# zahraamselim/compressed-rag-suite

Hardware: AMD Instinct MI355X
Metric: queries/sec over N-vector corpus (exact cosine top-k; Recall@10 vs the exact fp32 ranking) (higher is better)
Workload: dtype f16 x f16 -> f32; 1 GPU; c4; corpus_rows=10000000, rows_per_gpu=10000000, dim=384, queries_per_batch=64, distinct_queries_in_flight=2048, lanes=1 encoder + 1 search (encoder kernels <= 48 KB of LDS); 4 batches per sweep, batches_per_encoder_forward=16, searches_per_graph=4, top_k=10, k_scan=24, slab=f16, refine_fp32=True, exact_escalation=True, encoder_in_step=True, engine=rag._engine.RetrievalEngine (the object ContextRetriever.retrieve_batch drives), encoder=all-MiniLM-L6-v2 shape, seeded random weights

## Files before the change

### compressed-rag-suite_amd/csrc/capi.hip

```cpp
#include "../../include/crs_hip.h"

#include <hip/hip_runtime.h>
#include <stdio.h>
#include <string.h>

#include "plan.h"
#include "scan.h"

namespace crs {
int device_cus() {
  static int cus[64] = {0};
  int dev = 0;
  if (hipGetDevice(&dev) != hipSuccess) return 0;
  if (dev < 0 || dev >= 64) return 256;
  if (cus[dev] == 0) {
    hipDeviceProp_t p;
    if (hipGetDeviceProperties(&p, dev) != hipSuccess) return 0;
    cus[dev] = p.multiProcessorCount > 0 ? p.multiProcessorCount : 256;
  }
  return cus[dev];
}
}

namespace {
// ... 54 lines not shown
  const hipError_t e = hipGetLastError();
  return e == hipSuccess ? CRS_OK : hip_fail(e, what);
}
}

extern "C" {

const char* crs_last_error(void) { return g_err; }
int crs_abi_version(void) { return 3; }
int crs_row_elems(int dim, int slab_type) { return crs::row_elems(dim, slab_type); }
int crs_padded_dim(int dim) { return crs_row_elems(dim, CRS_SLAB_F16); }

int crs_scan_workspace_bytes(int nq, int dim, int k, int64_t n_rows, size_t* bytes) {
  if (!bytes) return fail(CRS_EINVAL, "null pointer");
  const char* why = "";
  const int rc = crs::plan_workspace_bytes(nq, dim, k, n_rows, device_cus(), crs::knobs_from_env(), bytes, &why);
  return rc ? fail(rc, "%s", why) : CRS_OK;
}

static int run_scan(const Plan& p, const void* q16, const void* slab, const float* scales, int64_t n_rows, const ScanWs& ws, hipStream_t st) {
  if (p.share_tau) {
    const hipError_t me = hipMemsetAsync(ws.tau, 0, ws.tau_bytes, st);
    if (me != hipSuccess) return (int)me;
  }
  crs::ScanArgs a;
  a.q = reinterpret_cast<const _Float16*>(q16);
  a.slab = slab;
  a.scales = scales;
  a.part_scores = ws.part_s;
  a.part_rows = ws.part_r;
  a.tau_shared = p.share_tau ? ws.tau : nullptr;
  a.stamps = nullptr;
  a.n_rows = (int)n_rows;
  a.n_tiles = p.n_tiles;
  a.nq = p.nq;
  a.k = p.k;
  a.sched = p.sched;
  a.boot = p.boot;
  a.kp = p.kp;
  a.nwg = p.nwg;
  a.nqb = p.nqb;
  a.ticket = p.ticket ? ws.tau : nullptr;
  a.t_dyn = p.t_dyn;
  a.dyn_mask = p.dyn_mask;
  a.nt = p.nt;
  a.no_stagger = p.no_stagger;
  a.no_defer = p.no_defer;
  if (p.ticket) {
    const int ze = crs::scan_ticket_zero(a.ticket, st);
    if (ze) return ze;
  }
  switch (p.family) {
    case crs::Family::W1: return crs::scan_launch_w1(a, p.pdim, st);
    case crs::Family::Wide: return crs::scan_launch_wide(a, p.pdim, p.waves, p.mfma, st);
    default: break;
  }
  if (p.slab_type == CRS_SLAB_I8) return crs::scan_launch_i8(a, p.pdim, p.slots, st);
  return p.family == crs::Family::TileBest ? crs::scan_launch_tb(a, p.pdim, p.waves, p.slots, st) : crs::scan_launch_f16(a, p.pdim, p.variant, st);
}

static int search_args_ok(const Plan& p, const void* q16_dev, const void* slab_dev, const float* scales_dev,
                          const void* workspace_dev, size_t workspace_bytes, const void* out_scores_dev, const void* out_ids_dev) {
  if (!q16_dev || !slab_dev || !workspace_dev || !out_scores_dev || !out_ids_dev)
    return fail(CRS_EINVAL, "null pointer");
  if (p.slab_type == CRS_SLAB_I8 && !scales_dev) return fail(CRS_EINVAL, "int8 slab needs scales");
  if (((uintptr_t)q16_dev | (uintptr_t)slab_dev) & 15) return fail(CRS_EINVAL, "q/slab must be 16-byte aligned");
  if (workspace_bytes < ws_bytes(p)) return fail(CRS_ENOSPC, "workspace too small");
  return CRS_OK;
}

int crs_cosine_topk(const void* q16_dev, int nq, int dim, int slab_type, const void* slab_dev,
                    const float* scales_dev, int64_t n_rows, int k, int64_t id_base,
                    void* workspace_dev, size_t workspace_bytes, float* out_scores_dev,
                    int64_t* out_ids_dev, void* stream) {
  if (slab_type != CRS_SLAB_F16 && slab_type != CRS_SLAB_I8) return fail(CRS_EINVAL, "bad slab_type");
  Plan p;
  int rc = plan_for(nq, dim, k, n_rows, slab_type, &p);
  if (rc) return rc;
  rc = search_args_ok(p, q16_dev, slab_dev, scales_dev, workspace_dev, workspace_bytes, out_scores_dev, out_ids_dev);
  if (rc) return rc;
  hipStream_t st = (hipStream_t)stream;
  ScanWs w = scan_ws(workspace_dev, p);
  int e = run_scan(p, q16_dev, slab_dev, scales_dev, n_rows, w, st);
  if (e == -1) return fail(CRS_EINVAL, "unsupported padded dimension");
  if (e) return hip_fail((hipError_t)e, "scan launch");
  if ((size_t)crs::merge_slices(p.nwg, p.kp) > crs::inter_lists(p.part_elems, nq)) w.inter_s = nullptr;
  if (!p.group_best()) {
    e = crs::merge_launch_i32(w.part_s, w.part_r, p.nwg, nq, p.kp, k, id_base, out_scores_dev, out_ids_dev, w.inter_s, w.inter_i, st);
    if (e) return hip_fail((hipError_t)e, "merge launch");
    return CRS_OK;
  }
  e = crs::merge_launch_i32(w.part_s, w.part_r, p.nwg, nq, p.kp, k, 0, w.win_s, w.win_i, w.inter_s, w.inter_i, st);
  if (e) return hip_fail((hipError_t)e, "merge launch");
  e = (slab_type == CRS_SLAB_I8)
          ? crs::refine_i8_launch(reinterpret_cast<const _Float16*>(q16_dev), nq, p.pdim, slab_dev, scales_dev, (int)n_rows, w.win_s,
                                  w.win_i, k, p.tile_rows, id_base, out_scores_dev, out_ids_dev, st)
          : crs::refine_launch(reinterpret_cast<const _Float16*>(q16_dev), nq, p.pdim, reinterpret_cast<const _Float16*>(slab_dev),
                               (int)n_rows, w.win_s, w.win_i, k, p.tile_rows, id_base, out_scores_dev, out_ids_dev, st);
  if (e == -1) return fail(CRS_EINVAL, "unsupported padded dimension");
  if (e) return hip_fail((hipError_t)e, "refine launch");
  return CRS_OK;
}

int crs_merge_topk(const float* scores_dev, const int64_t* ids_dev, int nlists, int nq, int k_in,
                   int k_out, float* out_scores_dev, int64_t* out_ids_dev, void* stream) {
  if (nlists <= 0 || nq <= 0 || k_in <= 0 || k_out <= 0 || k_out > CRS_MAX_K) return fail(CRS_EINVAL, "bad sizes (k_out <= CRS_MAX_K)");
  if (!scores_dev || !ids_dev || !out_scores_dev || !out_ids_dev) return fail(CRS_EINVAL, "null pointer");
// ... 521 lines not shown
```

### compressed-rag-suite_amd/csrc/plan.cpp

```cpp
#include "plan.h"

#include <stdio.h>
#include <stdlib.h>

#include "../../include/crs_hip.h"

namespace crs {
namespace {

bool env_on(const char* name) {
  const char* e = getenv(name);
  return !(e && e[0] == '0');
}
int env_digit(const char* name, int hi, int dflt) {
  const char* e = getenv(name);
  return (e && e[0] >= '0' && e[0] <= '0' + hi) ? e[0] - '0' : dflt;
}

Knobs read_once() {
  Knobs kn;
  kn.scan_tb = env_on("CRS_SCAN_TB");
  kn.long_chain = env_on("CRS_SCAN_LONG_CHAIN");
  kn.scan_wide = env_on("CRS_SCAN_WIDE");
  kn.scan_w1 = env_on("CRS_SCAN_W1");
  kn.scan_variant = env_digit("CRS_SCAN_VARIANT", 3, 3);
  kn.share_tau = env_digit("CRS_SCAN_SHARE_TAU", 1, 0) == 1;
  kn.scan_boot = env_on("CRS_SCAN_BOOT");
  kn.scan_sched = env_digit("CRS_SCAN_SCHED", 2, 2);
  return kn;
}

size_t align_up(size_t x, size_t a) { return (x + a - 1) / a * a; }

int partial_width(const Knobs& kn, int k) { return (kn.share_tau && k <= 16) ? 16 : k; }

void lay_out(Plan* p, int64_t n_rows, int cus, int tile_rows, int wg_per_cu, int queries) {
  p->tile_rows = tile_rows;
  p->n_tiles = (int)((n_rows + tile_rows - 1) / tile_rows);
  p->nqb = (p->nq + queries - 1) / queries;
  int streams = cus * wg_per_cu / p->nqb;
  if (streams < 1) streams = 1;
  if (p->nqb > 1 && streams >= 8) streams &= ~7;
  p->nwg = p->n_tiles < streams ? p->n_tiles : streams;
  if (p->nqb > 1 && p->nwg >= 8) p->nwg &= ~7;
}
int tiles_per_stream(const Plan& p) { return (p.n_tiles + p.nwg - 1) / p.nwg; }

int tile_best_slots(const Plan& p, const Knobs& kn) {
  const int tps = tiles_per_stream(p);
  if ((size_t)tps * p.nwg <= 8192 && tps <= 2 * scan_wide_slots(p.k)) return 0;
  if (p.k <= 16) return scan_wide_slots(p.k);
  const int slots = !kn.long_chain ? 0
                    : p.slab_type == CRS_SLAB_I8 ? scan_i8_long_chain_slots(p.pdim, p.k) : scan_tb_long_chain_slots(p.pdim, p.waves, p.k);
  return slots > 0 ? slots : -1;
}

int finish_plan(Plan* p, int64_t n_rows, const Knobs& kn) {
  const bool tile_best = p->family == Family::TileBest, wide = p->family == Family::Wide;
  p->part_elems = (size_t)p->nwg * p->nq * p->kp;
  p->share_tau = kn.share_tau;
  const size_t slab_bytes = (size_t)n_rows * p->pdim * (p->slab_type == CRS_SLAB_I8 ? 1 : 2);
  const bool streamed = tile_best || (wide && scan_wide_streamed(p->k));
  p->nt = !streamed ? 0 : kn.scan_nt >= 0 ? kn.scan_nt : (slab_bytes >= ((size_t)1 << 30) && p->nqb == 1);
  const bool tb_chain = tile_best && p->slots > 0 && !(p->slab_type == CRS_SLAB_I8 && p->pdim > 768);
  const bool wide_chain = wide && scan_wide_streamed(p->k) && kn.wide_dyn;
  const int rounds = p->n_tiles / p->nwg;
  p->ticket = (tb_chain || wide_chain) && p->nqb == 1 && !kn.share_tau && kn.tb_dyn > 0 &&
              rounds >= (kn.tb_dyn_min < 4 ? 4 : kn.tb_dyn_min);
  p->t_dyn = p->n_tiles;
  p->dyn_mask = 0;
  if (p->ticket) {
    int stat = (int)((int64_t)rounds * (100 - kn.tb_dyn) / 100);
    if (stat < 2) stat = 2;
    p->t_dyn = stat * p->nwg;
    p->dyn_mask = kn.tb_dyn_g - 1;
  }
  p->boot = (kn.scan_boot && rounds < 24) ? 1 : 0;
  p->sched = kn.scan_sched;
  p->no_stagger = (wide && !kn.wide_stagger) ? 1 : 0;
  p->no_defer = (wide && !kn.wide_defer) ? 1 : 0;
  p->mfma = !wide ? 0 : !wide_has_16(p->pdim, p->waves, p->slots) ? 32 : kn.wide_mfma ? kn.wide_mfma : wide_default_mfma(p->pdim, p->slots);
  return CRS_OK;
}

}

Knobs knobs_from_env() {
  static const Knobs once = read_once();
  Knobs kn = once;
  if (const char* e = getenv("CRS_TB_DYN")) { const int v = atoi(e); kn.tb_dyn = v < 0 ? 0 : v > 100 ? 100 : v; }
  if (const char* e = getenv("CRS_TB_DYN_G")) { const int v = atoi(e); kn.tb_dyn_g = v >= 16 ? 16 : v >= 8 ? 8 : v >= 4 ? 4 : v >= 2 ? 2 : 1; }
  if (const char* e = getenv("CRS_TB_DYN_MIN")) kn.tb_dyn_min = atoi(e);
  kn.wide_dyn = env_on("CRS_WIDE_DYN");
  kn.scan_nt = env_digit("CRS_SCAN_NT", 1, -1);
  kn.fused_tail = env_on("CRS_FUSED_TAIL");
  kn.wide_stagger = env_on("CRS_WIDE_STAGGER");
  kn.wide_defer = env_on("CRS_WIDE_DEFER");
  const char* me = getenv("CRS_WIDE_MFMA");
  kn.wide_mfma = !me ? 0 : (me[0] == '1' && me[1] == '6' && !me[2]) ? 16 : (me[0] == '3' && me[1] == '2' && !me[2]) ? 32 : 0;
  return kn;
}

bool Plan::form_exists() const {
  switch (family) {
    case Family::W1: return w1_form_exists(pdim);
    case Family::Wide: return wide_form_exists(pdim, waves, slots, mfma);
    case Family::TileBest: return slab_type == CRS_SLAB_I8 ? i8_form_exists(pdim, slots) : tb_form_exists(pdim, waves, slots);
    default: return slab_type == CRS_SLAB_I8 ? i8_form_exists(pdim, -1) : classic_form_exists(pdim, classic_list_slots(k));
  }
}

int make_plan(int nq, int dim, int k, int64_t n_rows, int slab_type, int cus, const Knobs& kn, Plan* p, const char** why) {
  const auto bad = [&](int code, const char* msg) { *why = msg; return code; };
  if (nq <= 0 || dim <= 0 || dim > 1024) return bad(CRS_EINVAL, "nq must be > 0 and 0 < dim <= 1024");
  if (k <= 0 || k > CRS_MAX_K) return bad(CRS_EINVAL, "k must be in 1..CRS_MAX_K");
  if (n_rows <= 0 || n_rows > 0x7fffffffLL - 64) return bad(CRS_EINVAL, "n_rows must be in 1..2^31-65");
  if (cus <= 0) return bad(CRS_EHIP, "no HIP device available");
  const bool f16 = slab_type == CRS_SLAB_F16;
  const int pdim = row_elems(dim, slab_type);
  *p = Plan{};
  p->slab_type = slab_type;
  p->nq = nq;
  p->k = k;
  p->pdim = pdim;
  p->variant = kn.scan_variant;

  if (kn.scan_tb && kn.scan_w1 && f16 && nq > 64 && w1_form_exists(pdim)) {
    p->family = Family::W1;
    p->waves = 8;
    lay_out(p, n_rows, cus, kW1TileRows, kW1WgPerCu, kW1Queries);
    p->kp = tiles_per_stream(*p);
    if (p->kp <= kW1MaxDump) return finish_plan(p, n_rows, kn);
  }
  if (kn.scan_tb && kn.scan_wide && f16 && nq > 64 && wide_serves(k, pdim)) {
    p->family = Family::Wide;
    p->waves = nq > 128 ? 8 : 4;
    p->slots = scan_wide_slots(k);
    lay_out(p, n_rows, cus, scan_wide_tile_rows(p->waves, pdim), scan_wide_wg_per_cu(p->waves), wide_queries(p->waves));
    p->kp = 2 * p->slots;
    return finish_plan(p, n_rows, kn);
  }
  if (kn.scan_tb) {
    p->family = Family::TileBest;
    if (f16) {
      p->waves = (nq > 64 && k <= 16 && scan_tb_has_8_waves(pdim)) ? 8 : 4;
      lay_out(p, n_rows, cus, tb_tile_rows(pdim), tb_wg_per_cu(pdim, p->waves), tb_queries(p->waves));
    } else {
      p->waves = 4;
      lay_out(p, n_rows, cus, i8_tile_rows(), classic_wg_per_cu(kn.scan_variant), kI8Queries);
    }
// ... 60 lines not shown
```

### compressed-rag-suite_amd/csrc/plan.h

```cpp
#pragma once
#include <stddef.h>
#include <stdint.h>

#include "scan_forms.h"

namespace crs {

struct Knobs {
  bool scan_tb = true;
  bool long_chain = true;
  bool scan_wide = true;
  bool scan_w1 = true;
  int scan_variant = 3;
  bool share_tau = false;
  bool scan_boot = true;
  int scan_sched = 2;
  int tb_dyn = 85;
  int tb_dyn_g = 8;
  int tb_dyn_min = 96;
  bool wide_dyn = true;
  int scan_nt = -1;
  bool fused_tail = true;
  bool wide_stagger = true;
  bool wide_defer = true;
  int wide_mfma = 0;
};
Knobs knobs_from_env();

constexpr int kW1MaxDump = 256;

struct Plan {
  Family family;
  int slab_type;
  int nq, k;
  int pdim, tile_rows, n_tiles;
  int nwg;
  int nqb;
  int kp;
  int waves;
  int slots;
  int variant;
  bool share_tau;
  int nt;
  bool ticket;
  int t_dyn, dyn_mask;
  int boot, sched;
  int no_stagger;
  int no_defer;
  int mfma;
  size_t part_elems;
  bool group_best() const { return family != Family::Classic; }
  bool form_exists() const;
};

int make_plan(int nq, int dim, int k, int64_t n_rows, int slab_type, int cus, const Knobs& kn, Plan* p, const char** why);
int plan_describe(const Plan& p, char* buf, size_t cap);

struct WsLayout {
  size_t tau, part_s, part_r, win_s, win_i, inter_s, inter_i;
  size_t tau_bytes, bytes;
};
size_t inter_lists(size_t part_elems, int nq);
WsLayout ws_layout(size_t part_elems, int nq, int k);
int plan_workspace_bytes(int nq, int dim, int k, int64_t n_rows, int cus, const Knobs& kn, size_t* bytes, const char** why);

}
```

### compressed-rag-suite_amd/csrc/scan.h

```cpp
#pragma once
#include <hip/hip_runtime.h>
#include <stdint.h>

#include "scan_forms.h"

namespace crs {

int set_error(int code, const char* msg);
int launch_status(const char* what);

struct ScanArgs {
  const _Float16* q;
  const void* slab;
  const float* scales;
  float* part_scores;
  int* part_rows;
  unsigned* tau_shared;
  unsigned long long* stamps;
  int n_rows;
  int n_tiles;
  int nq;
  int k;
  int sched;
  int boot;
  int kp;
  int nwg;
  int nqb;
  unsigned* ticket;
  int t_dyn;
  int dyn_mask;
  int nt;
  int no_stagger;
  int no_defer;
};

struct ExactWs {
  float* thr;
  int* cnt;
  int* done;
  int64_t* lists;
};

int refine_launch(const _Float16* q16, int nq, int pdim, const _Float16* slab, int n_rows, const float* win_s,
                  const int64_t* win, int k, int tile_rows, int64_t id_base, float* out_s, int64_t* out_i, hipStream_t stream);

int refine_i8_launch(const _Float16* q16, int nq, int pdim, const void* slab, const float* scales, int n_rows, const float* win_s,
                     const int64_t* win, int k, int tile_rows, int64_t id_base, float* out_s, int64_t* out_i, hipStream_t stream);

int scan_launch_f16(const ScanArgs& a, int pdim, int variant, hipStream_t stream);
int scan_launch_i8(const ScanArgs& a, int pdim, int slots, hipStream_t stream);
int scan_launch_tb(const ScanArgs& a, int pdim, int nw, int slots, hipStream_t stream);
int scan_ticket_zero(unsigned* ticket, hipStream_t stream);
int scan_launch_wide(const ScanArgs& a, int pdim, int nw, int mfma, hipStream_t stream);
int scan_launch_w1(const ScanArgs& a, int pdim, hipStream_t stream);

int merge_slices(int nlists, int k_in);
int merge_launch_i32(const float* scores, const int* rows, int nlists, int nq, int k_in, int k_out,
                     int64_t id_base, float* out_scores, int64_t* out_ids, float* inter_s, int64_t* inter_i, hipStream_t stream);
int merge_launch_i64(const float* scores, const int64_t* ids, int nlists, int nq, int k_in, int k_out,
                     float* out_scores, int64_t* out_ids, hipStream_t stream);

int merge_launch_wire(const void* wire, size_t block_bytes, size_t scores_off, int nlists, int nq, int k_in, int k_out,
                      float* out_scores, int64_t* out_ids, hipStream_t stream);

int merge_sorted_launch_i64(const float* scores, const int64_t* ids, int nlists, int nq, int k_in, int k_out, float* out_scores,
                            int64_t* out_ids, hipStream_t stream);
int merge_sorted_launch_wire(const void* wire, size_t block_bytes, size_t scores_off, int nlists, int nq, int k_in, int k_out,
                             float* out_scores, int64_t* out_ids, hipStream_t stream);

int mmr_order_launch(const float* vecs, int64_t n_rows, int dim, const int64_t* rows, const double* rel, const int* counts, int nq,
                     int m_max, double lam, int* order, hipStream_t stream);

int rerank_lexical_launch(const float* scores, const int64_t* rows, int nq, int m_max, const int64_t* doc_off, const int* doc_tok,
                          int64_t n_rows, int64_t n_doc_tok, const int64_t* q_off, const int* q_tok, int64_t n_q_tok, const int* q_norm,
                          int k, double threshold, int* order, int* out_count, double* sim, double* rr, int* reranked, hipStream_t stream);

size_t bm25_workspace_bytes(int nq, int k, int64_t n_rows);
int bm25_topk_launch(const int64_t* doc_off, const int* doc_tok, const int* doc_tf, const int* doc_len, int64_t n_rows, int64_t n_doc_tok,
                     const int64_t* q_off, const int* q_tok, const float* q_w, int nq, int n_pairs, float c0, float c1, float k1p1, int k,
                     void* workspace, float* out_s, int64_t* out_i, hipStream_t stream);

int fuse_rrf_launch(const int64_t* dense, int m_dense, const int64_t* lex, int m_lex, int nq, double c, double w_dense, double w_lex,
                    int k_out, int64_t* out_rows, double* out_fused, int* out_dpos, int* out_lpos, int* out_count, hipStream_t stream);

int wordpiece_encode_launch(const uint8_t* text, const int64_t* offsets, int n_texts, int64_t n_bytes, const uint32_t* table,
                            int64_t table_len, const uint32_t* rep, int64_t rep_len, const int32_t* slots, int64_t n_slots,
                            const uint32_t* pool, int64_t pool_len, int max_probe, int lmax, int mode, int unk, int cls, int sep, int pad,
                            int hash_lo, int hash_span, int max_len, int* ids, int* lens, int* flags, hipStream_t stream);
int unigram_encode_launch(const uint8_t* text, const int64_t* offsets, int n_texts, int64_t n_bytes, const uint32_t* table,
                          int64_t table_len, const uint32_t* rep, int64_t rep_len, const int32_t* slots, const double* slot_scores,
                          int64_t n_slots, const uint32_t* pool, int64_t pool_len, int max_probe, int lmax, double unk_score, int opts,
                          int unk, int cls, int sep, int pad, int max_len, int* ids, int* lens, int* flags, hipStream_t stream);

int token_match_launch(const float* a, const int* len_a, int seq_a, const float* b, const int* len_b, int seq_b, int n_pairs, int hidden,
                       const float* w_a, const float* w_b, float* out, hipStream_t stream);

int pairs_above_launch(const void* slab, int pdim, int64_t a_first, int64_t a_rows, int64_t b_first, int64_t b_rows, float thr,
                       int64_t* pairs_out, float* scores_out, int64_t cap, int64_t* counter, hipStream_t stream);
int pairs_verify_launch(const int64_t* pairs, int64_t m, const float* shadow, int64_t n_rows, int d, float thr, int64_t* rows_a,
                        int64_t* rows_b, float* sims, int64_t* counter, hipStream_t stream);

int refine_f32_launch(const float* q32, int nq, int dim, const float* shadow, int64_t n_rows, int64_t id_base,
                      const int64_t* cand, int k_in, int k_out, float* out_s, int64_t* out_i, hipStream_t stream);
int score_rows_launch(const float* q32, int nq, int dim, const float* shadow, int64_t n_rows, int64_t id_base, int k, const int64_t* ids,
                      float* scores, hipStream_t stream);
int rescore_launch(const float* q32, int nq, int dim, const float* shadow, int64_t n_rows,
// ... 24 lines not shown
```

### compressed-rag-suite_amd/csrc/scan_forms.h

```cpp
#pragma once

namespace crs {

enum class Family { Classic, TileBest, Wide, W1 };

constexpr int kSlabF16 = 0, kSlabI8 = 1;

constexpr int row_elems(int dim, int slab_type) {
  const int g = slab_type == kSlabI8 ? 256 : 128;
  return dim <= 0 ? 0 : (dim + g - 1) / g * g;
}
constexpr bool f16_row(int pdim) { return pdim >= 128 && pdim <= 1024 && pdim % 128 == 0; }

constexpr int classic_wg_per_cu(int variant) { return variant == 1 ? 1 : 2; }
constexpr int classic_tile_rows(int pdim) { return pdim <= 512 ? 32 : 16; }
constexpr int classic_list_slots(int k) { return k <= 16 ? 16 : 32; }
constexpr int kClassicQueries = 64;
constexpr bool classic_form_exists(int pdim, int list_slots) { return f16_row(pdim) && (list_slots == 16 || list_slots == 32); }

constexpr int tb_tile_rows(int pdim) { return classic_tile_rows(pdim); }
constexpr bool scan_tb_has_8_waves(int pdim) { return pdim != 640 && pdim != 896; }
constexpr int tb_wg_per_cu(int pdim, int nw) { return nw == 8 ? (pdim <= 384 ? 2 : 1) : (pdim <= 128 ? 3 : 2); }
constexpr int tb_queries(int nw) { return 16 * nw; }
constexpr int scan_wide_slots(int k) { return k <= 4 ? 4 : k <= 10 ? 10 : k <= 16 ? 16 : k <= 24 ? 24 : 32; }
constexpr int scan_tb_long_chain_slots(int pdim, int nw, int k) {
  if (nw != 4 || k <= 16 || k > 64) return 0;
  if (k <= 24) return 24;
  if (k <= 32) return 32;
  if (pdim == 256) return 64;
  if (pdim == 384) return k <= 48 ? 48 : (k <= 56 ? 56 : 0);
  if (pdim == 512 || pdim == 640) return k <= 48 ? 48 : 0;
  if (pdim == 768) return k <= 40 ? 40 : 0;
  return 0;
}
constexpr bool tb_form_exists(int pdim, int nw, int slots) {
  if (!f16_row(pdim) || !(nw == 4 || (nw == 8 && scan_tb_has_8_waves(pdim)))) return false;
  if (slots == 0 || slots == 4 || slots == 10 || slots == 16) return true;
  return slots > 16 && scan_tb_long_chain_slots(pdim, nw, slots) == slots;
}

constexpr int i8_tile_rows() { return 32; }
constexpr int kI8Queries = 64;
constexpr int scan_i8_long_chain_slots(int pdim, int k) { return (k <= 16 || k > 48) ? 0 : k <= 32 ? 32 : (pdim <= 768 ? 48 : 0); }
constexpr bool i8_form_exists(int pdim, int slots) {
  if (!(pdim == 256 || pdim == 512 || pdim == 768 || pdim == 1024)) return false;
  if (slots == -1 || slots == 0 || slots == 4 || slots == 10 || slots == 16) return true;
  return slots > 16 && scan_i8_long_chain_slots(pdim, slots) == slots;
}

constexpr bool wide_serves(int k, int pdim) { return k <= 32 && pdim <= 512 && !(k > 16 && pdim > 384); }
constexpr int scan_wide_tile_rows(int nw, int pdim) { return (nw == 8 && pdim <= 384) ? 64 : 32; }
constexpr int scan_wide_wg_per_cu(int nw) { return nw == 8 ? 1 : 2; }
constexpr int wide_queries(int nw) { return 32 * nw; }
constexpr bool scan_wide_streamed(int k) { return scan_wide_slots(k) > 16; }
constexpr bool wide_has_16(int pdim, int nw, int slots) { return nw == 8 && (pdim == 256 || pdim == 384) && slots > 16; }
constexpr int wide_default_mfma(int pdim, int slots) { return (pdim == 384 && (slots == 24 || slots == 32)) ? 16 : 32; }
constexpr bool wide_form_exists(int pdim, int nw, int slots, int mfma) {
  if (!(pdim == 128 || pdim == 256 || pdim == 384 || pdim == 512) || !(nw == 4 || nw == 8)) return false;
  if (!(slots == 4 || slots == 10 || slots == 16 || ((slots == 24 || slots == 32) && pdim <= 384))) return false;
  return mfma == 32 || (mfma == 16 && wide_has_16(pdim, nw, slots));
}

constexpr int kW1TileRows = 32, kW1WgPerCu = 1, kW1Queries = 256;
constexpr bool w1_form_exists(int pdim) { return pdim == 768; }

}
```

### compressed-rag-suite_amd/csrc/scan_stream.h

```cpp
#pragma once
#include "scan_common.h"

namespace crs {
namespace {

typedef __attribute__((address_space(3))) void* lds_ptr_t;

__device__ __forceinline__ unsigned tile_lds_wave(char* tile_buf, int wave) {
  return __builtin_amdgcn_readfirstlane((unsigned)(size_t)(lds_ptr_t)tile_buf + (unsigned)wave * 1024u);
}

template <int kT, int kTileBytes, int kLoads>
__device__ __forceinline__ void stream_tile(const char* slab, int tile, int n_full, size_t last_chunk, unsigned dst0,
                                            const unsigned (&src_off)[kLoads], int nt) {
  if (tile < n_full) {
    const char* base = uniform_ptr(slab + (size_t)tile * kTileBytes);
    if (nt) {
#pragma unroll
      for (int j = 0; j < kLoads; ++j) lds_dma16_nt(dst0 + (unsigned)(j * kT * 16), src_off[j], base);
    } else {
#pragma unroll
      for (int j = 0; j < kLoads; ++j) lds_dma16(dst0 + (unsigned)(j * kT * 16), src_off[j], base);
    }
  } else {
#pragma unroll
    for (int j = 0; j < kLoads; ++j) {
      size_t off = (size_t)tile * kTileBytes + src_off[j];
      off = off > last_chunk ? last_chunk : off;
      const char* p = slab + off;
      const unsigned dst = dst0 + (unsigned)(j * kT * 16);
      lds_dma16(dst, p);
    }
  }
}

template <int K>
__device__ __forceinline__ void chain_insert(float (&ts)[K], int (&tr)[K], float x, int xr) {
#pragma unroll
  for (int j = 0; j < K; ++j) {
    const bool c = x > ts[j];
    const float s_old = ts[j];
    const int r_old = tr[j];
    ts[j] = c ? x : s_old;
    tr[j] = c ? xr : r_old;
    x = c ? s_old : x;
    xr = c ? r_old : xr;
  }
}

__device__ __forceinline__ bool ticket_due(bool in_dyn, int tn, int tstep, int t_dyn, int dyn_mask) {
  return in_dyn ? ((tn - t_dyn) & dyn_mask) == dyn_mask : tn + tstep >= t_dyn;
}
__device__ __forceinline__ void ticket_draw(unsigned& tk, bool drawer, unsigned* ticket) {
  const unsigned mask = __builtin_amdgcn_readfirstlane(drawer ? 1u : 0u);
  unsigned long long keep;
  unsigned zero = 0u, one = 1u;
  asm volatile("s_mov_b64 %1, exec\n\ts_mov_b32 exec_lo, %2\n\ts_mov_b32 exec_hi, 0\n\tglobal_atomic_add %0, %3, %4, %5 sc0\n\ts_mov_b64 exec, %1"
               : "+v"(tk), "=&s"(keep) : "s"(mask), "v"(zero), "v"(one), "s"(ticket) : "memory");
}
__device__ __forceinline__ void ticket_publish(int* sh_next, int it, unsigned tk, int t_dyn, int dyn_mask) {
  sh_next[it & 1] = t_dyn + (int)tk * (dyn_mask + 1);
}
__device__ __forceinline__ int ticket_take(const int* sh_next, int it, int tend) {
  const int tnn = __builtin_amdgcn_readfirstlane(sh_next[it & 1]);
  return (unsigned)tnn < (unsigned)tend ? tnn : tend;
}

__device__ __forceinline__ void dump_pad(float* part_s, int* part_r, size_t o, int first, int kp) {
  for (int p = first; p < kp; p += 4) {
    part_s[o + p] = kNegInf;
    part_r[o + p] = -1;
  }
}
template <int K>
__device__ __forceinline__ void chain_store(float* part_s, int* part_r, size_t o, const float (&ts)[K], const int (&tr)[K]) {
#pragma unroll
  for (int j = 0; j < K; ++j) {
    part_s[o + j] = ts[j];
    part_r[o + j] = tr[j];
  }
}

template <auto kKernel>
int launch_scan(int lds, int threads, const ScanArgs& a, hipStream_t stream) {
  static bool done = false;
  if (!done) {
    hipError_t e = hipFuncSetAttribute(reinterpret_cast<const void*>(kKernel), hipFuncAttributeMaxDynamicSharedMemorySize, lds);
    if (e != hipSuccess) return (int)e;
    done = true;
  }
  hipLaunchKernelGGL(kKernel, dim3(a.nqb * a.nwg), dim3(threads), lds, stream, a);
  return (int)hipGetLastError();
}

}
}
```

### compressed-rag-suite_amd/csrc/scan_wide.hip

```cpp


#include "scan_stream.h"

namespace crs {
namespace {

typedef float f32x16 __attribute__((ext_vector_type(16)));

template <int D, int NW>
constexpr int wide_rb() { return scan_wide_tile_rows(NW, D) / 32; }

template <int K>
constexpr bool wide_streamed() { return K > 16; }
template <int K>
constexpr bool wide_split() { return K > 16; }
template <int K>
constexpr int wide_lane_slots() { return wide_split<K>() ? K / 2 : K; }
template <int D, int NW, int K>
constexpr bool wide_stagger() {
  if (D == 384 && NW == 8 && K == 24) return true;
  return NW == 8 && D <= 384 && !(D == 384 && K >= 16) && !(D == 256 && K >= 32);
}
#ifndef CRS_WIDE_DEFER_ALL
#define CRS_WIDE_DEFER_ALL 0
#endif
template <int D, int NW, int K, bool S16>
constexpr bool wide_defer() {
  if (!wide_split<K>() || (!S16 && D == 384 && NW == 8 && K == 24)) return false;
  if (CRS_WIDE_DEFER_ALL) return true;
  return S16 && D == 384 && NW == 8 && K == 24;
}

template <int D, int NW>
struct WCfg {
  static constexpr int kThreadsW = NW * 64;
  static constexpr int kCpr = D / 8;
  static constexpr int RB = wide_rb<D, NW>();
  static constexpr int TR = 32 * RB;
  static constexpr int kTileBytes = TR * D * 2;
  static constexpr int kLoads = kTileBytes / (kThreadsW * 16);
  static constexpr int kKsteps = D / 16;
  static constexpr int kQStage = NW * 4096;
  static constexpr int kLds = 2 * kTileBytes > kTileBytes + kQStage ? 2 * kTileBytes : kTileBytes + kQStage;
  static_assert(D % 128 == 0, "row length must be a multiple of 128 elements");
  static_assert(kTileBytes % (kThreadsW * 16) == 0, "tile must split into whole 16-byte loads");
};

template <int RB, bool S16>
struct WAcc { f32x16 a[RB]; };
template <int RB>
struct WAcc<RB, true> { f32x4 a[2 * RB][2]; };

template <int D, int NW, int K, bool S16>
__device__ __forceinline__ void scan_wide_body(const ScanArgs a) {
  using C = WCfg<D, NW>;
  static_assert(!S16 || wide_has_16(D, NW, K), "the 16x16x32 form exists for the split-list forms of 64-row tiles only");
  constexpr int kT = C::kThreadsW;
  extern __shared__ __attribute__((aligned(16))) char smem[];
  char* tile_buf = smem;
  const int tid = threadIdx.x;
  const int lane = tid & 63;
  const int wave = __builtin_amdgcn_readfirstlane(tid >> 6);
  const int nwg = CRS_NSTREAMS;
  const int qblock = CRS_QBLOCK, stream = CRS_STREAM;
  WP_DECL;
  const bool wave_active = (qblock * (NW * 32) + wave * 32) < a.nq;

  unsigned src_off[C::kLoads];
#pragma unroll
  for (int j = 0; j < C::kLoads; ++j) {
    const int P = j * kT + tid;
    const int r = P / C::kCpr, cp = P % C::kCpr;
    src_off[j] = (unsigned)(r * C::kCpr + ((cp & ~15) | ((cp ^ r) & 15))) * 16u;
  }
  const char* slab = reinterpret_cast<const char*>(a.slab);
  const size_t last_chunk = (size_t)a.n_rows * (D * 2) - 16;
  constexpr int RB = C::RB, WTR = C::TR;
  const int n_full = a.n_rows / WTR;
  const unsigned lds_wave = tile_lds_wave(tile_buf, wave);
  auto dma_tile = [&](int tile, int buf) {
    stream_tile<kT, C::kTileBytes>(slab, __builtin_amdgcn_readfirstlane(tile), n_full, last_chunk,
                                   lds_wave + (unsigned)(buf * C::kTileBytes), src_off, wide_streamed<K>() ? a.nt : 0);
  };

  __shared__ int sh_next[2];
  constexpr bool kDyn = wide_streamed<K>();
  const int tend = a.n_tiles;
  const int t_dyn = kDyn ? a.t_dyn : a.n_tiles;
  int t = stream, t_prev = stream;
  int tn = t + nwg;
  dma_tile(t, 0);

  constexpr int KS16 = D / 32;
  const int kq = lane >> 4;
  const int qn = S16 ? (lane & 15) : (lane & 31), h = S16 ? (kq & 1) : (lane >> 5);
  const int qi = qblock * (NW * 32) + wave * 32 + (S16 ? 16 * (kq >> 1) : 0) + qn;
  const bool q_valid = qi < a.nq;
  f16x8 qf[C::kKsteps];
  {
    constexpr int kBlocks = C::kCpr / 8;
    constexpr int kGroup = 3;
    char* qs = tile_buf + C::kTileBytes + wave * 4096;
    const int q0 = qblock * (NW * 32) + wave * 32;
    const char* qbytes = reinterpret_cast<const char*>(a.q);
    const f16x8 z = {0, 0, 0, 0, 0, 0, 0, 0};
#pragma unroll
    for (int g0 = 0; g0 < kBlocks; g0 += kGroup) {
      u32x4 tmp[kGroup * 4];
#pragma unroll
      for (int p = 0; p < kGroup; ++p) {
        if (g0 + p < kBlocks) {
#pragma unroll
          for (int j = 0; j < 4; ++j) {
            const int c = j * 64 + lane, q = c >> 3, col = c & 7;
            const int qq = q0 + q < a.nq ? q0 + q : a.nq - 1;
            tmp[p * 4 + j] = *reinterpret_cast<const u32x4*>(qbytes + (size_t)qq * (D * 2) + (g0 + p) * 128 + col * 16);
          }
        }
      }
#pragma unroll
      for (int p = 0; p < kGroup; ++p) {
        if (g0 + p < kBlocks) {
#pragma unroll
          for (int j = 0; j < 4; ++j) {
            const int c = j * 64 + lane, q = c >> 3, col = c & 7;
            *reinterpret_cast<u32x4*>(qs + q * 128 + ((col ^ ((q >> 1) & 7)) * 16)) = tmp[p * 4 + j];
          }
          if constexpr (S16) {
#pragma unroll
            for (int g = 0; g < 2; ++g) {
              const int row = 16 * g + qn;
#pragma unroll
              for (int kk = 0; kk < 2; ++kk) {
                const int col = 4 * kk + kq;
                const f16x8 v = *reinterpret_cast<const f16x8*>(qs + row * 128 + ((col ^ ((row >> 1) & 7)) * 16));
                qf[g * KS16 + (g0 + p) * 2 + kk] = (q0 + row < a.nq) ? v : z;
              }
            }
          } else {
#pragma unroll
            for (int ksl = 0; ksl < 4; ++ksl) {
              const int col = 2 * ksl + h;
              const f16x8 v = *reinterpret_cast<const f16x8*>(qs + qn * 128 + ((col ^ ((qn >> 1) & 7)) * 16));
              qf[(g0 + p) * 4 + ksl] = q_valid ? v : z;
            }
          }
        }
      }
    }
#pragma unroll
    for (int ks = 0; ks < C::kKsteps; ++ks) {
      f16x8 x = qf[ks];
      asm volatile("" : "+v"(x));
      qf[ks] = x;
    }
// ... 130 lines not shown
#pragma unroll
          for (int rt = 0; rt < 2 * RB; rt += 2) xg[g] = __builtin_fmaxf(__builtin_fmaxf(xg[g], m[rt]), m[rt + 1]);
        } else {
#pragma unroll
          for (int rt = 0; rt < 2 * RB; ++rt) {
            const int row0 = te * WTR + 16 * rt + 4 * kq;
#pragma unroll
            for (int i = 0; i < 4; ++i) xg[g] = (row0 + i < a.n_rows) ? __builtin_fmaxf(xg[g], accs.a[rt][g][i]) : xg[g];
          }
        }
      }
      const auto r0 = __builtin_amdgcn_permlane16_swap(__float_as_uint(xg[0]), __float_as_uint(xg[0]), false, false);
      const auto r1 = __builtin_amdgcn_permlane16_swap(__float_as_uint(xg[1]), __float_as_uint(xg[1]), false, false);
      const float y0 = __builtin_fmaxf(__uint_as_float(r0[0]), __uint_as_float(r0[1]));
      const float y1 = __builtin_fmaxf(__uint_as_float(r1[0]), __uint_as_float(r1[1]));
      const auto rr = __builtin_amdgcn_permlane32_swap(__float_as_uint(y0), __float_as_uint(y1), false, false);
      x = __builtin_fmaxf(__uint_as_float(rr[0]), __uint_as_float(rr[1]));
      pair_tile(x, te * WTR);
    } else {
#pragma unroll
      for (int rb = 0; rb < RB; ++rb) {
        const f32x16& acc = accs.a[rb];
        if (te < n_full) {
          const float m0 = __builtin_fmaxf(__builtin_fmaxf(acc[0], acc[1]), acc[2]);
          const float m1 = __builtin_fmaxf(__builtin_fmaxf(acc[3], acc[4]), acc[5]);
          const float m2 = __builtin_fmaxf(__builtin_fmaxf(acc[6], acc[7]), acc[8]);
          const float m3 = __builtin_fmaxf(__builtin_fmaxf(acc[9], acc[10]), acc[11]);
          const float m4 = __builtin_fmaxf(__builtin_fmaxf(acc[12], acc[13]), acc[14]);
          x = __builtin_fmaxf(x, __builtin_fmaxf(__builtin_fmaxf(__builtin_fmaxf(m0, m1), __builtin_fmaxf(m2, m3)), __builtin_fmaxf(m4, acc[15])));
        } else {
          const int row_base = te * WTR + rb * 32 + 4 * h;
#pragma unroll
          for (int r = 0; r < 16; ++r) {
            const int row = row_base + 8 * (r >> 2) + (r & 3);
            x = (row < a.n_rows) ? __builtin_fmaxf(x, acc[r]) : x;
          }
        }
      }
      x = pair_max(x);
      if constexpr (kSplit) {
        pair_tile(x, te * WTR);
      } else {
        if ((ie & 1) == h) { px = x; pr = te * WTR; }
        if (ie & 1) {
          chain_insert(ts, tr, px, pr);
          px = kNegInf;
          pr = -1;
        }
      }
    }
  };

  int cur = 0, it = 0;
  while (t < tend) {
    const bool has_next = tn < tend;
    if (has_next) dma_tile(tn, cur ^ 1);
    const bool in_dyn = kDyn && tn >= t_dyn;
    const bool draw = kDyn && a.ticket != nullptr && has_next && ticket_due(in_dyn, tn, nwg, t_dyn, a.dyn_mask);
    unsigned tk = 0;
    if constexpr (kDyn) ticket_draw(tk, draw && wave == 0, a.ticket);
    if (wave_active) {
      WP_LAP(1);
      const char* buf = tile_buf + cur * C::kTileBytes;
      if (!late) {
        const Acc acc = sweep(buf);
        WP_LAP(3);
        select(acc, t, it);
      } else {
        if (it > 0) select(acc_prev, t_prev, it - 1);
        WP_LAP(2);
        acc_prev = sweep(buf);
        WP_LAP(3);
      }
    }
    WP_LAP(4);
    int tnn = in_dyn ? tn + 1 : tn + nwg;
    if constexpr (kDyn) {
      asm volatile("s_waitcnt vmcnt(0)" : "+v"(tk) : : "memory");
      if (draw && tid == 0) ticket_publish(sh_next, it, tk, t_dyn, a.dyn_mask);
    } else {
      asm volatile("s_waitcnt vmcnt(0)" ::: "memory");
    }
    WP_LAP(6);
    __syncthreads();
    WP_LAP(7);
    if (kDyn && draw) tnn = ticket_take(sh_next, it, tend);
    cur ^= 1;
    ++it;
    t_prev = t;
    t = tn;
    tn = tnn;
  }

  if (wave_active && late && it > 0) select(acc_prev, t_prev, it - 1);
  if constexpr (kSplit) {
    if constexpr (kDefer) {
      if (wave_active) flush();
    }
    if (wave_active && q_valid) {
      const size_t o = ((size_t)qi * nwg + stream) * a.kp + (size_t)h * KL;
#pragma unroll
      for (int j = 0; j < KL; ++j) {
        a.part_scores[o + j] = ts[j];
        a.part_rows[o + j] = tr[j];
        a.part_scores[o + K + j] = kNegInf;
        a.part_rows[o + K + j] = -1;
      }
    }
  } else {
    if (wave_active && (it & 1)) chain_insert(ts, tr, px, pr);
    if (wave_active && q_valid) {
      const size_t o = ((size_t)qi * nwg + stream) * a.kp + (size_t)h * K;
#pragma unroll
      for (int j = 0; j < K; ++j) {
        a.part_scores[o + j] = ts[j];
        a.part_rows[o + j] = tr[j];
      }
    }
  }
  WP_LAP(10);
  WP_STORE(NW);
}

template <int D, int NW, int K>
__global__ __launch_bounds__(NW * 64, 2) void scan_wide_kernel(const ScanArgs a) {
  scan_wide_body<D, NW, K, false>(a);
}
template <int D, int NW, int K>
__global__ __launch_bounds__(NW * 64, 2) void scan_wide16_kernel(const ScanArgs a) {
  scan_wide_body<D, NW, K, true>(a);
}

template <int D, int NW, int K, bool S16>
int launch_wide(const ScanArgs& a, hipStream_t stream) {
  if constexpr (S16) return launch_scan<&scan_wide16_kernel<D, NW, K>>(WCfg<D, NW>::kLds, NW * 64, a, stream);
  else return launch_scan<&scan_wide_kernel<D, NW, K>>(WCfg<D, NW>::kLds, NW * 64, a, stream);
}

template <int D, int NW, int K>
int launch_wide_if(const ScanArgs& a, int mfma, hipStream_t stream) {
  if constexpr (wide_form_exists(D, NW, K, 16)) {
    if (mfma == 16) return launch_wide<D, NW, K, true>(a, stream);
  }
  if constexpr (wide_form_exists(D, NW, K, 32)) return launch_wide<D, NW, K, false>(a, stream);
  else return -1;
}

template <int D, int NW>
int launch_wide_k(const ScanArgs& a, int mfma, hipStream_t stream) {
  switch (scan_wide_slots(a.k)) {
    case 4: return launch_wide_if<D, NW, 4>(a, mfma, stream);
    case 10: return launch_wide_if<D, NW, 10>(a, mfma, stream);
    case 16: return launch_wide_if<D, NW, 16>(a, mfma, stream);
    case 24: return launch_wide_if<D, NW, 24>(a, mfma, stream);
    default: return launch_wide_if<D, NW, 32>(a, mfma, stream);
  }
}

template <int D>
int launch_wide_d(const ScanArgs& a, int nw, int mfma, hipStream_t stream) {
  return nw == 8 ? launch_wide_k<D, 8>(a, mfma, stream) : launch_wide_k<D, 4>(a, mfma, stream);
}

}

int scan_launch_wide(const ScanArgs& a, int pdim, int nw, int mfma, hipStream_t stream) {
  switch (pdim) {
    case 128: return launch_wide_d<128>(a, nw, mfma, stream);
    case 256: return launch_wide_d<256>(a, nw, mfma, stream);
    case 384: return launch_wide_d<384>(a, nw, mfma, stream);
    case 512: return launch_wide_d<512>(a, nw, mfma, stream);
    default: return -1;
  }
}

}
```

Baseline: 124,300 queries/s.

## Add triple-buffered ring pipeline to the wide scan kernel for pdim 384

Adds a three-buffer ring variant of the wide f16 scan kernel that keeps two tile DMAs in flight instead of one. The ticket-based dynamic scheduling is moved to per-slot shared slots so a tile index can be drawn two steps ahead. The goal is to hide more global-memory latency while streaming the slab. In exchange each workgroup uses more LDS, which may lower occupancy, and the static prefix is raised to at least three rounds. It is enabled by default only for pdim 384, 8 waves, 24 slots and the 16x16 MFMA form, and is compiled in a separate translation unit.

```diff
diff --git a/compressed-rag-suite_amd/csrc/capi.hip b/compressed-rag-suite_amd/csrc/capi.hip
--- a/compressed-rag-suite_amd/csrc/capi.hip
+++ b/compressed-rag-suite_amd/csrc/capi.hip
@@ -130,7 +130,8 @@
   }
   switch (p.family) {
     case crs::Family::W1: return crs::scan_launch_w1(a, p.pdim, st);
-    case crs::Family::Wide: return crs::scan_launch_wide(a, p.pdim, p.waves, p.mfma, st);
+    case crs::Family::Wide:
+      return p.ring ? crs::scan_launch_wide_ring(a, p.pdim, p.waves, p.mfma, st) : crs::scan_launch_wide(a, p.pdim, p.waves, p.mfma, st);
     default: break;
   }
   if (p.slab_type == CRS_SLAB_I8) return crs::scan_launch_i8(a, p.pdim, p.slots, st);
diff --git a/compressed-rag-suite_amd/csrc/plan.cpp b/compressed-rag-suite_amd/csrc/plan.cpp
--- a/compressed-rag-suite_amd/csrc/plan.cpp
+++ b/compressed-rag-suite_amd/csrc/plan.cpp
@@ -1,5 +1,6 @@
 #include "plan.h"
 
+#include <assert.h>
 #include <stdio.h>
 #include <stdlib.h>
 
@@ -65,21 +66,25 @@
   const bool tb_chain = tile_best && p->slots > 0 && !(p->slab_type == CRS_SLAB_I8 && p->pdim > 768);
   const bool wide_chain = wide && scan_wide_streamed(p->k) && kn.wide_dyn;
   const int rounds = p->n_tiles / p->nwg;
+  p->mfma = !wide ? 0 : !wide_has_16(p->pdim, p->waves, p->slots) ? 32 : kn.wide_mfma ? kn.wide_mfma : wide_default_mfma(p->pdim, p->slots);
+  p->ring = wide && kn.wide_ring && wide_ring_form(p->pdim, p->waves, p->slots, p->mfma);
+  p->lds = wide ? scan_wide_lds_bytes(p->pdim, p->waves, p->ring) : 0;
   p->ticket = (tb_chain || wide_chain) && p->nqb == 1 && !kn.share_tau && kn.tb_dyn > 0 &&
               rounds >= (kn.tb_dyn_min < 4 ? 4 : kn.tb_dyn_min);
   p->t_dyn = p->n_tiles;
   p->dyn_mask = 0;
   if (p->ticket) {
     int stat = (int)((int64_t)rounds * (100 - kn.tb_dyn) / 100);
-    if (stat < 2) stat = 2;
+    const int stat_min = p->ring ? 3 : 2;
+    if (stat < stat_min) stat = stat_min;
     p->t_dyn = stat * p->nwg;
     p->dyn_mask = kn.tb_dyn_g - 1;
+    assert(p->t_dyn >= stat_min * p->nwg && p->t_dyn <= p->n_tiles);
   }
   p->boot = (kn.scan_boot && rounds < 24) ? 1 : 0;
   p->sched = kn.scan_sched;
   p->no_stagger = (wide && !kn.wide_stagger) ? 1 : 0;
   p->no_defer = (wide && !kn.wide_defer) ? 1 : 0;
-  p->mfma = !wide ? 0 : !wide_has_16(p->pdim, p->waves, p->slots) ? 32 : kn.wide_mfma ? kn.wide_mfma : wide_default_mfma(p->pdim, p->slots);
   return CRS_OK;
 }
 
@@ -96,6 +101,7 @@
   kn.fused_tail = env_on("CRS_FUSED_TAIL");
   kn.wide_stagger = env_on("CRS_WIDE_STAGGER");
   kn.wide_defer = env_on("CRS_WIDE_DEFER");
+  kn.wide_ring = env_on("CRS_WIDE_RING");
   const char* me = getenv("CRS_WIDE_MFMA");
   kn.wide_mfma = !me ? 0 : (me[0] == '1' && me[1] == '6' && !me[2]) ? 16 : (me[0] == '3' && me[1] == '2' && !me[2]) ? 32 : 0;
   return kn;
diff --git a/compressed-rag-suite_amd/csrc/plan.h b/compressed-rag-suite_amd/csrc/plan.h
--- a/compressed-rag-suite_amd/csrc/plan.h
+++ b/compressed-rag-suite_amd/csrc/plan.h
@@ -24,6 +24,7 @@
   bool wide_stagger = true;
   bool wide_defer = true;
   int wide_mfma = 0;
+  bool wide_ring = true;
 };
 Knobs knobs_from_env();
 
@@ -48,6 +49,8 @@
   int no_stagger;
   int no_defer;
   int mfma;
+  bool ring;
+  int lds;
   size_t part_elems;
   bool group_best() const { return family != Family::Classic; }
   bool form_exists() const;
diff --git a/compressed-rag-suite_amd/csrc/scan.h b/compressed-rag-suite_amd/csrc/scan.h
--- a/compressed-rag-suite_amd/csrc/scan.h
+++ b/compressed-rag-suite_amd/csrc/scan.h
@@ -52,6 +52,7 @@
 int scan_launch_tb(const ScanArgs& a, int pdim, int nw, int slots, hipStream_t stream);
 int scan_ticket_zero(unsigned* ticket, hipStream_t stream);
 int scan_launch_wide(const ScanArgs& a, int pdim, int nw, int mfma, hipStream_t stream);
+int scan_launch_wide_ring(const ScanArgs& a, int pdim, int nw, int mfma, hipStream_t stream);
 int scan_launch_w1(const ScanArgs& a, int pdim, hipStream_t stream);
 
 int merge_slices(int nlists, int k_in);
diff --git a/compressed-rag-suite_amd/csrc/scan_forms.h b/compressed-rag-suite_amd/csrc/scan_forms.h
--- a/compressed-rag-suite_amd/csrc/scan_forms.h
+++ b/compressed-rag-suite_amd/csrc/scan_forms.h
@@ -61,6 +61,19 @@
   return mfma == 32 || (mfma == 16 && wide_has_16(pdim, nw, slots));
 }
 
+#ifndef CRS_WIDE_RING_ALL
+#define CRS_WIDE_RING_ALL 0
+#endif
+constexpr bool wide_ring_form(int pdim, int nw, int slots, int mfma) {
+  if (!wide_form_exists(pdim, nw, slots, mfma) || nw != 8 || slots <= 16) return false;
+  if (CRS_WIDE_RING_ALL) return true;
+  return pdim == 384 && slots == 24 && mfma == 16;
+}
+constexpr int scan_wide_lds_bytes(int pdim, int nw, bool ring) {
+  const int tile = scan_wide_tile_rows(nw, pdim) * pdim * 2, qstage = nw * 4096, nbuf = ring ? 3 : 2;
+  return nbuf * tile > (nbuf - 1) * tile + qstage ? nbuf * tile : (nbuf - 1) * tile + qstage;
+}
+
 constexpr int kW1TileRows = 32, kW1WgPerCu = 1, kW1Queries = 256;
 constexpr bool w1_form_exists(int pdim) { return pdim == 768; }
 
diff --git a/compressed-rag-suite_amd/csrc/scan_stream.h b/compressed-rag-suite_amd/csrc/scan_stream.h
--- a/compressed-rag-suite_amd/csrc/scan_stream.h
+++ b/compressed-rag-suite_amd/csrc/scan_stream.h
@@ -66,6 +66,14 @@
   return (unsigned)tnn < (unsigned)tend ? tnn : tend;
 }
 
+__device__ __forceinline__ void ticket_publish_slot(int* sh_next, int slot, unsigned tk, int t_dyn, int dyn_mask) {
+  sh_next[slot] = t_dyn + (int)tk * (dyn_mask + 1);
+}
+__device__ __forceinline__ int ticket_take_slot(const int* sh_next, int slot, int tend) {
+  const int tnn = __builtin_amdgcn_readfirstlane(sh_next[slot]);
+  return (unsigned)tnn < (unsigned)tend ? tnn : tend;
+}
+
 __device__ __forceinline__ void dump_pad(float* part_s, int* part_r, size_t o, int first, int kp) {
   for (int p = first; p < kp; p += 4) {
     part_s[o + p] = kNegInf;
diff --git a/compressed-rag-suite_amd/csrc/scan_wide.hip b/compressed-rag-suite_amd/csrc/scan_wide.hip
--- a/compressed-rag-suite_amd/csrc/scan_wide.hip
+++ b/compressed-rag-suite_amd/csrc/scan_wide.hip
@@ -30,6 +30,9 @@
   if (CRS_WIDE_DEFER_ALL) return true;
   return S16 && D == 384 && NW == 8 && K == 24;
 }
+
+template <int D, int NW, int K, bool S16>
+constexpr bool wide_ring() { return wide_ring_form(D, NW, K, S16 ? 16 : 32); }
 
 template <int D, int NW>
 struct WCfg {
@@ -42,6 +45,8 @@
   static constexpr int kKsteps = D / 16;
   static constexpr int kQStage = NW * 4096;
   static constexpr int kLds = 2 * kTileBytes > kTileBytes + kQStage ? 2 * kTileBytes : kTileBytes + kQStage;
+  static constexpr int kLdsRing = scan_wide_lds_bytes(D, NW, true);
+  static_assert(kLds == scan_wide_lds_bytes(D, NW, false), "the planner's LDS bytes are the launch's");
   static_assert(D % 128 == 0, "row length must be a multiple of 128 elements");
   static_assert(kTileBytes % (kThreadsW * 16) == 0, "tile must split into whole 16-byte loads");
 };
@@ -51,9 +56,10 @@
 template <int RB>
 struct WAcc<RB, true> { f32x4 a[2 * RB][2]; };
 
-template <int D, int NW, int K, bool S16>
+template <int D, int NW, int K, bool S16, bool RING = false>
 __device__ __forceinline__ void scan_wide_body(const ScanArgs a) {
   using C = WCfg<D, NW>;
+  static_assert(!RING || (wide_ring<D, NW, K, S16>() && wide_streamed<K>()), "no ring kernel for this form");
   static_assert(!S16 || wide_has_16(D, NW, K), "the 16x16x32 form exists for the split-list forms of 64-row tiles only");
   constexpr int kT = C::kThreadsW;
   extern __shared__ __attribute__((aligned(16))) char smem[];
@@ -83,13 +89,16 @@
                                    lds_wave + (unsigned)(buf * C::kTileBytes), src_off, wide_streamed<K>() ? a.nt : 0);
   };
 
-  __shared__ int sh_next[2];
+  __shared__ int sh_next[RING ? 3 : 2];
   constexpr bool kDyn = wide_streamed<K>();
   const int tend = a.n_tiles;
   const int t_dyn = kDyn ? a.t_dyn : a.n_tiles;
   int t = stream, t_prev = stream;
   int tn = t + nwg;
   dma_tile(t, 0);
+  if constexpr (RING) {
+    if (tn < tend) dma_tile(tn, 1);
+  }
 
   constexpr int KS16 = D / 32;
   const int kq = lane >> 4;
@@ -100,7 +109,7 @@
   {
     constexpr int kBlocks = C::kCpr / 8;
     constexpr int kGroup = 3;
-    char* qs = tile_buf + C::kTileBytes + wave * 4096;
+    char* qs = tile_buf + (RING ? 2 : 1) * C::kTileBytes + wave * 4096;
     const int q0 = qblock * (NW * 32) + wave * 32;
     const char* qbytes = reinterpret_cast<const char*>(a.q);
     const f16x8 z = {0, 0, 0, 0, 0, 0, 0, 0};
@@ -337,6 +346,55 @@
   };
 
   int cur = 0, it = 0;
+  if constexpr (RING) {
+    int tnn = tn + nwg;
+    while (t < tend) {
+      const bool has_nn = tnn < tend;
+      const int nbuf = cur ? cur - 1 : 2;
+      const bool in_dyn = tnn >= t_dyn;
+      const bool draw = a.ticket != nullptr && has_nn && ticket_due(in_dyn, tnn, nwg, t_dyn, a.dyn_mask);
+      unsigned tk = 0;
+      ticket_draw(tk, draw && wave == 0, a.ticket);
+      auto issue = [&]() {
+        WP_LAP(6);
+        if (has_nn) dma_tile(tnn, nbuf);
+        WP_LAP(1);
+      };
+      const char* buf = tile_buf + cur * C::kTileBytes;
+      if (!wave_active) {
+        asm volatile("s_waitcnt vmcnt(0)" ::: "memory");
+        issue();
+      } else if (!late) {
+        const Acc acc = sweep(buf);
+        WP_LAP(3);
+        select(acc, t, it);
+        WP_LAP(4);
+        asm volatile("s_waitcnt vmcnt(0)" : "+v"(tk) : : "memory");
+        issue();
+        if (draw && tid == 0) ticket_publish_slot(sh_next, cur, tk, t_dyn, a.dyn_mask);
+      } else {
+        if (it > 0) select(acc_prev, t_prev, it - 1);
+        WP_LAP(2);
+        asm volatile("s_waitcnt vmcnt(0)" ::: "memory");
+        issue();
+        acc_prev = sweep(buf);
+        WP_LAP(3);
+      }
+      int t3 = in_dyn ? tnn + 1 : tnn + nwg;
+      asm volatile("s_waitcnt lgkmcnt(0)" ::: "memory");
+      __builtin_amdgcn_s_barrier();
+      asm volatile("" ::: "memory");
+      WP_LAP(7);
+      if (draw) t3 = ticket_take_slot(sh_next, cur, tend);
+      cur = cur == 2 ? 0 : cur + 1;
+      ++it;
+      t_prev = t;
+      t = tn;
+      tn = tnn;
+      tnn = t3;
+    }
+    asm volatile("s_waitcnt vmcnt(0)" ::: "memory");
+  } else {
   while (t < tend) {
     const bool has_next = tn < tend;
     if (has_next) dma_tile(tn, cur ^ 1);
@@ -376,6 +434,7 @@
     t = tn;
     tn = tnn;
   }
+  }
 
   if (wave_active && late && it > 0) select(acc_prev, t_prev, it - 1);
   if constexpr (kSplit) {
@@ -407,6 +466,11 @@
   WP_STORE(NW);
 }
 
+#ifndef CRS_WIDE_TU
+#define CRS_WIDE_TU 0
+#endif
+
+#if CRS_WIDE_TU != 1
 template <int D, int NW, int K>
 __global__ __launch_bounds__(NW * 64, 2) void scan_wide_kernel(const ScanArgs a) {
   scan_wide_body<D, NW, K, false>(a);
@@ -447,8 +511,44 @@
   return nw == 8 ? launch_wide_k<D, 8>(a, mfma, stream) : launch_wide_k<D, 4>(a, mfma, stream);
 }
 
-}
-
+#endif
+
+#if CRS_WIDE_TU != 0
+namespace ring {
+template <int D, int NW, int K>
+__global__ __launch_bounds__(NW * 64, 2) void scan_wide_kernel(const ScanArgs a) {
+  scan_wide_body<D, NW, K, false, true>(a);
+}
+template <int D, int NW, int K>
+__global__ __launch_bounds__(NW * 64, 2) void scan_wide16_kernel(const ScanArgs a) {
+  scan_wide_body<D, NW, K, true, true>(a);
+}
+}
+
+template <int D, int K>
+int launch_ring_if(const ScanArgs& a, int mfma, hipStream_t stream) {
+  if constexpr (wide_ring<D, 8, K, true>()) {
+    if (mfma == 16) return launch_scan<&ring::scan_wide16_kernel<D, 8, K>>(WCfg<D, 8>::kLdsRing, 8 * 64, a, stream);
+  }
+  if constexpr (wide_ring<D, 8, K, false>()) {
+    if (mfma == 32) return launch_scan<&ring::scan_wide_kernel<D, 8, K>>(WCfg<D, 8>::kLdsRing, 8 * 64, a, stream);
+  }
+  return -1;
+}
+
+template <int D>
+int launch_ring_d(const ScanArgs& a, int mfma, hipStream_t stream) {
+  switch (scan_wide_slots(a.k)) {
+    case 24: return launch_ring_if<D, 24>(a, mfma, stream);
+    case 32: return launch_ring_if<D, 32>(a, mfma, stream);
+    default: return -1;
+  }
+}
+#endif
+
+}
+
+#if CRS_WIDE_TU != 1
 int scan_launch_wide(const ScanArgs& a, int pdim, int nw, int mfma, hipStream_t stream) {
   switch (pdim) {
     case 128: return launch_wide_d<128>(a, nw, mfma, stream);
@@ -458,5 +558,18 @@
     default: return -1;
   }
 }
-
-}
+#endif
+
+#if CRS_WIDE_TU != 0
+int scan_launch_wide_ring(const ScanArgs& a, int pdim, int nw, int mfma, hipStream_t stream) {
+  if (nw != 8) return -1;
+  switch (pdim) {
+    case 128: return launch_ring_d<128>(a, mfma, stream);
+    case 256: return launch_ring_d<256>(a, mfma, stream);
+    case 384: return launch_ring_d<384>(a, mfma, stream);
+    default: return -1;
+  }
+}
+#endif
+
+}
diff --git a/compressed-rag-suite_amd/csrc/scan_wide_ring.hip b/compressed-rag-suite_amd/csrc/scan_wide_ring.hip
--- /dev/null
+++ b/compressed-rag-suite_amd/csrc/scan_wide_ring.hip
@@ -0,0 +1,2 @@
+#define CRS_WIDE_TU 1
+#include "scan_wide.hip"
```

Result: faster. 128,500 queries/s (median of 6 runs) (+3.4%).
